# KrArunT/whisper-rust-ort

Measured on AMD Instinct MI355X. Metric: rtfx: audio seconds transcribed per wall second (whisper-base, 30 s clips, greedy 128 new tokens), higher is better.
Workload: dtype bf16

## Files before the change

### whisper-rust-ort_amd/build.py

```python
from __future__ import annotations

import os
import subprocess
import sys
from concurrent.futures import ThreadPoolExecutor

HERE = os.path.dirname(os.path.abspath(__file__))
CSRC = os.path.join(HERE, "csrc")
OUT = os.path.join(HERE, "libwhisper_hip.so")
SOURCES = ["wh_mel.hip", "wh_gemm.hip", "wh_gemm8.hip", "wh_gemm8x.hip", "wh_gemm8_mx.hip", "wh_mlp.hip", "wh_attn.hip", "wh_decode.hip", "wh_dec_tile.hip", "wh_cross_es.hip", "wh_cross_es8.hip", "wh_cross_es3.hip", "wh_fp8.hip", "wh_align.hip", "wh_model.cpp", "wh_api.cpp"]
HEADERS = ["wh_common.h", "wh_es_common.h", "wh_kernels.h", "wh_lm_tile.h", "wh_internal.h", "wh_json.h", "../../include/whisper_hip.h"]
FLAGS = ["--offload-arch=gfx950", "-O3", "-fPIC", "-std=c++17", "-pthread", "-Wall", "-Wno-unused-function", "-Wno-unused-value", "-Wno-unused-result",
         "-mllvm", "-amdgpu-mfma-vgpr-form=1", "-x", "hip"]


EXTRA_FLAGS = {"wh_attn.hip": ["-fno-honor-nans"], "wh_cross_es.hip": ["-fno-honor-nans"], "wh_cross_es8.hip": ["-fno-honor-nans"], "wh_cross_es3.hip": ["-fno-honor-nans"]}


def _stale(target: str, deps) -> bool:
    if not os.path.exists(target):
        return True
    t = os.path.getmtime(target)
    return any(os.path.getmtime(d) > t for d in deps)


def build(verbose: bool = False, force: bool = False) -> str:
    hipcc = os.environ.get("HIPCC", "/opt/rocm/bin/hipcc")
    objdir = os.path.join(HERE, "build")
    os.makedirs(objdir, exist_ok=True)
    hdrs = [os.path.join(CSRC, h) for h in HEADERS]

    def compile_one(src: str) -> str:
        s = os.path.join(CSRC, src)
        o = os.path.join(objdir, src + ".o")
        if force or _stale(o, [s] + hdrs):
            cmd = [hipcc] + FLAGS + EXTRA_FLAGS.get(src, []) + ["-c", s, "-o", o]
            if verbose:
                print(" ".join(cmd), flush=True)
            subprocess.check_call(cmd)
        return o

    with ThreadPoolExecutor(max_workers=min(6, os.cpu_count() or 1)) as ex:
        objs = list(ex.map(compile_one, SOURCES))
    if force or _stale(OUT, objs):
        cmd = [hipcc, "--offload-arch=gfx950", "-shared", "-fPIC", "-pthread", "-o", OUT] + objs
        if verbose:
            print(" ".join(cmd), flush=True)
        subprocess.check_call(cmd)
    build_host(verbose, force)
    build_tools(verbose, force)
    return OUT


TOOLS = os.path.join(HERE, "..", "tools")


def build_tools(verbose: bool = False, force: bool = False) -> None:
    hipcc = os.environ.get("HIPCC", "/opt/rocm/bin/hipcc")
    for name, kernel_src in (("mx_mfma_check", "wh_gemm8_mx.hip"), ("mx_gemm_check", "wh_gemm8_mx.hip"), ("mlp_check", "wh_mlp.hip"), ("es16_check", "wh_cross_es.hip"), ("es8_check", "wh_cross_es8.hip"), ("es3_check", "wh_cross_es3.hip"), ("align_check", "wh_align.hip")):
        src, exe = os.path.join(TOOLS, name + ".hip"), os.path.join(TOOLS, name)
        deps = [src, os.path.join(CSRC, kernel_src), os.path.join(CSRC, "wh_common.h"), os.path.join(CSRC, "wh_es_common.h"), os.path.join(CSRC, "wh_kernels.h")]
        if force or _stale(exe, deps):
            cmd = [hipcc, "--offload-arch=gfx950", "-O3", "-std=c++17", "-mllvm", "-amdgpu-mfma-vgpr-form=1"] + EXTRA_FLAGS.get(kernel_src, []) + ["-w", "-I", CSRC, src, "-o", exe]
            if verbose:
                print(" ".join(cmd), flush=True)
            subprocess.check_call(cmd)


HOST = os.path.join(HERE, "host")
HOST_SO = os.path.join(HERE, "libwh_host.so")
CLI = os.path.join(HERE, "whisper_bench")


def build_host(verbose: bool = False, force: bool = False) -> None:
    gxx = os.environ.get("CXX", "g++")
    hdr = [os.path.join(HOST, "wh_host.h"), os.path.join(HOST, "wh_unicode_lower.h"), os.path.join(CSRC, "wh_json.h"), os.path.join(HERE, "..", "include", "whisper_hip.h")]
    src = os.path.join(HOST, "wh_host_capi.cpp")
    if force or _stale(HOST_SO, [src] + hdr):
        cmd = [gxx, "-O2", "-std=c++17", "-fPIC", "-shared", "-Wall", "-o", HOST_SO, src]
        if verbose:
            print(" ".join(cmd), flush=True)
        subprocess.check_call(cmd)
    src = os.path.join(HOST, "whisper_bench.cpp")
    if force or _stale(CLI, [src, OUT] + hdr):
        cmd = [gxx, "-O2", "-std=c++17", "-Wall", "-pthread", "-D__HIP_PLATFORM_AMD__", "-I/opt/rocm/include", "-o", CLI, src, "-L" + HERE, "-lwhisper_hip",
               "-Wl,-rpath,$ORIGIN", "-Wl,-rpath,/opt/rocm/lib", "-L/opt/rocm/lib", "-lamdhip64"]
        if verbose:
            print(" ".join(cmd), flush=True)
        subprocess.check_call(cmd)


if __name__ == "__main__":
    print(build(verbose=True, force="--force" in sys.argv))
```

### whisper-rust-ort_amd/csrc/wh_decode.hip

```cpp
#include <stdlib.h>

#include "wh_common.h"
#include "wh_kernels.h"

#include <algorithm>
#include <mutex>
#include <unordered_map>

int wh_dbg_cross_unroll = 4;
int wh_dbg_lm_blocks_per_cu = 2;
int wh_dbg_lm_mt = 4;
int wh_dbg_mt = 0;
int wh_dbg_nw = 0;
int wh_dbg_wide = -1;

namespace {

__device__ __forceinline__ void advance_if_last(int* ticket, int* pos_p, int n_blocks) {
    if (!ticket) return;
    __syncthreads();
    if (threadIdx.x == 0) {
        const int t = atomicAdd(ticket, 1);
        if (t == n_blocks - 1) {
            *ticket = 0;
// ... 895 lines not shown
    const int fl = lane & 15, fg = lane >> 4;
    const int n_tiles = (a.n_lang + 15) >> 4;
    const int m0 = blockIdx.y * MT * 16;
    T* Xs = reinterpret_cast<T*>(smem_raw);
    constexpr int ROWS = MT * 16;
    const int nslab = a.K >> 5, cps = ROWS * 32 / EPC;
    u32x4 xr[16];
    int xo[16];
    auto stage_load = [&](int c0) {
#pragma unroll
        for (int i = 0; i < 16; i++) {
            const int c = min(c0 + i * 256, nslab * cps - 1), sl = c / cps, o = (c - sl * cps) * EPC;
            xo[i] = sl * ROWS * 32 + o;
            xr[i] = *reinterpret_cast<const u32x4*>((const T*)a.X + ((long)sl * a.x_mpad + m0) * 32 + o);
        }
    };
    auto stage_store = [&](int c0) {
#pragma unroll
        for (int i = 0; i < 16; i++)
            if (c0 + i * 256 < nslab * cps) *reinterpret_cast<u32x4*>(Xs + xo[i]) = xr[i];
    };
    stage_load(tid);
    float* lnstat = reinterpret_cast<float*>(smem_raw + (size_t)nslab * ROWS * 32 * sizeof(T));
    {
        float* lnq = lnstat + 2 * ROWS;
        if (tid < 4 * ROWS) {
            const int r = tid % ROWS, q = tid / ROWS;
            float s1, s2;
            ln_partial_sum(a.ln_part, a.ln_tiles, a.x_mpad, m0 + r, q, 4, s1, s2);
            lnq[(q * ROWS + r) * 2] = s1;
            lnq[(q * ROWS + r) * 2 + 1] = s2;
        }
        __syncthreads();
        if (tid < ROWS) {
            const float s1 = (lnq[tid * 2] + lnq[(ROWS + tid) * 2]) + (lnq[(2 * ROWS + tid) * 2] + lnq[(3 * ROWS + tid) * 2]);
            const float s2 = (lnq[tid * 2 + 1] + lnq[(ROWS + tid) * 2 + 1]) + (lnq[(2 * ROWS + tid) * 2 + 1] + lnq[(3 * ROWS + tid) * 2 + 1]);
            float mean, rstd;
            wh_ln_mean_rstd(s1, s2, (float)a.K, false, mean, rstd);
            lnstat[2 * tid] = mean;
            lnstat[2 * tid + 1] = rstd;
        }
    }
    const int iters = a.K >> 5;
    constexpr int DEPTH = sizeof(typename FragT<T>::type) <= 16 ? 16 : 8;
    const int nchunk = (iters + DEPTH - 1) / DEPTH;
    const int tile = blockIdx.x * 4 + wave;
    const int units = tile < n_tiles ? nchunk : 0;
    typedef typename FragT<T>::type frag_t;
    frag_t wA[DEPTH], wB[DEPTH];
    f32x4 acc[MT];
#pragma unroll
    for (int t = 0; t < MT; t++) acc[t] = f32x4{0, 0, 0, 0};
    const T* wp = (const T*)a.W + (long)a.ids[min(tile, WH_LANG_LD / 16 - 1) * 16 + fl] * a.K + fg * 8;
    auto load_unit = [&](frag_t (&wq)[DEPTH], int u) {
#pragma unroll
        for (int i = 0; i < DEPTH; i++)
            if (u * DEPTH + i < iters) wq[i] = load_frag<T>(wp + (u * DEPTH + i) * 32);
    };
    auto compute_unit = [&](const frag_t (&wq)[DEPTH], int u) {
#pragma unroll
        for (int i = 0; i < DEPTH; i++) {
            if (u * DEPTH + i < iters) {
#pragma unroll
                for (int t = 0; t < MT; t++) {
                    frag_t xf = load_frag<T>(Xs + ((long)(u * DEPTH + i) * ROWS + t * 16 + fl) * 32 + fg * 8);
                    mma16(acc[t], wq[i], xf);
                }
            }
        }
    };
    if (units > 0) load_unit(wA, 0);
    stage_store(tid);
    for (int c0 = tid + 256 * 16; c0 < nslab * cps; c0 += 256 * 16) {
        stage_load(c0);
        stage_store(c0);
    }
    __syncthreads();
    for (int u = 0; u < units; u += 2) {
        const bool hasB = u + 1 < units;
        if (hasB) load_unit(wB, u + 1);
        compute_unit(wA, u);
        if (hasB) {
            if (u + 2 < units) load_unit(wA, u + 2);
            compute_unit(wB, u + 1);
        }
    }
    if (units == 0) return;
    const int j0 = tile * 16 + 4 * fg;
    float sv[4] = {0, 0, 0, 0}, cv[4] = {0, 0, 0, 0};
#pragma unroll
    for (int e = 0; e < 4; e++) {
        const int id = a.ids[j0 + e];
        sv[e] = a.ln_s[id];
        cv[e] = a.bias[id];
    }
#pragma unroll
    for (int t = 0; t < MT; t++) {
        const int m = m0 + t * 16 + fl;
        const float mean = lnstat[2 * (t * 16 + fl)], rstd = lnstat[2 * (t * 16 + fl) + 1];
        f32x4 v;
#pragma unroll
        for (int e = 0; e < 4; e++) v[e] = wh_ln_fold(acc[t][e], mean, rstd, sv[e], cv[e]);
        if (m < a.M) *reinterpret_cast<f32x4*>(a.out + (long)m * WH_LANG_LD + j0) = v;
    }
}

__global__ __launch_bounds__(64) void k_lang_finish(const float* __restrict__ logits, const int* __restrict__ ids, int n_lang, int src_row,
                                                    float* __restrict__ probs, int* __restrict__ chosen, int* __restrict__ feed,
                                                    int* __restrict__ out_tokens, int tok_ld, int tok_pos, int* pos_p) {
    const int b = blockIdx.x, lane = threadIdx.x;
    const float* row = logits + (long)(src_row >= 0 ? src_row : b) * WH_LANG_LD;
    float v[2];
    int id[2];
    float bv = -INFINITY;
    int bi = 0x7fffffff, lo = 0x7fffffff;
#pragma unroll
    for (int k = 0; k < 2; k++) {
        const int j = lane + 64 * k;
        const bool in = j < n_lang;
        v[k] = in ? row[j] : NAN;
        id[k] = in ? ids[j] : 0x7fffffff;
        lo = min(lo, id[k]);
        if (v[k] > bv || (v[k] == bv && id[k] < bi)) { bv = v[k]; bi = id[k]; }
    }
#pragma unroll
    for (int off = 32; off > 0; off >>= 1) {
        const float ov = __shfl_xor(bv, off);
        const int oi = __shfl_xor(bi, off), ol = __shfl_xor(lo, off);
        if (ov > bv || (ov == bv && oi < bi)) { bv = ov; bi = oi; }
        lo = min(lo, ol);
    }
    const bool none = bv == -INFINITY;
    float e[2], s = 0.0f;
#pragma unroll
    for (int k = 0; k < 2; k++) {
        e[k] = (none || !(v[k] == v[k])) ? 0.0f : (bv == INFINITY ? (v[k] == INFINITY ? 1.0f : 0.0f) : ts_exp(v[k] - bv));
        s += e[k];
    }
    s = wave_sum(s);
#pragma unroll
    for (int k = 0; k < 2; k++) {
        const int j = lane + 64 * k;
        if (j < n_lang) probs[(long)b * n_lang + j] = none ? 0.0f : e[k] / s;
    }
    if (lane == 0) {
        const int tok = none ? lo : bi;
        chosen[b] = tok;
        feed[(long)b * tok_ld + tok_pos] = tok;
        out_tokens[(long)b * tok_ld + tok_pos] = tok;
        if (pos_p && b == 0) *pos_p += 1;
    }
}

template <typename T, typename TO = T, bool PFX = false>
__global__ __launch_bounds__(64) void k_dec_self_attn(const T* __restrict__ qkv, T* __restrict__ kc,
                                                      T* __restrict__ vc, TO* __restrict__ out,
                                                      const int* __restrict__ pos_p, int d, int n_heads, int tc_plane,
                                                      int mpad, const int* __restrict__ off) {
    constexpr int HD = WH_HEAD_DIM;
    typedef typename FragT<T>::type frag_t;
    __shared__ __attribute__((aligned(16))) float qs[HD];
    __shared__ __attribute__((aligned(16))) float sc[512];
    const int h = blockIdx.x, b = blockIdx.y, lane = threadIdx.x, gpos = *pos_p;
    int adv = 0;
    if constexpr (PFX) adv = min(max(off[b], 0), gpos);
    const int pos = gpos - adv, tc = tc_plane - adv;
    const T* row = qkv + (long)b * 3 * d;
    T* kcb = kc + (((long)b * n_heads + h) * tc_plane + adv) * HD;
    T* vcb = vc + (((long)b * n_heads + h) * tc_plane + adv) * HD;
    frag_t kr[2][HD / 8];
#pragma unroll
    for (int i = 0; i < 2; i++) {
        const int j = lane + 64 * i;
        if (j < pos) {
#pragma unroll
            for (int e = 0; e < HD / 8; e++) kr[i][e] = load_frag<T>(kcb + (long)j * HD + e * 8);
        }
    }
    constexpr int EPC = 16 / (int)sizeof(T), CPR = HD / EPC, RPI = 64 / CPR, NPRE = 8;
    typedef __attribute__((ext_vector_type(EPC))) T vrow_t;
    const int rslot = lane / CPR, chunk = lane % CPR;
    vrow_t vpre[NPRE];
#pragma unroll
    for (int u = 0; u < NPRE; u++)
        vpre[u] = *reinterpret_cast<const vrow_t*>(vcb + (long)min(u * RPI + rslot, tc - 1) * HD + chunk * EPC);
    const vrow_t vcur_v = *reinterpret_cast<const vrow_t*>(row + 2 * d + h * HD + chunk * EPC);
    const T kcur = row[d + h * HD + lane], vcur = row[2 * d + h * HD + lane];
    qs[lane] = cvt_in<T>(row[h * HD + lane]);
    kcb[(long)pos * HD + lane] = kcur;
    vcb[(long)pos * HD + lane] = vcur;
    __syncthreads();
    float mx = -INFINITY;
#pragma unroll
    for (int i = 0; i < 2; i++) {
        const int j = lane + 64 * i;
        if (j < pos) {
            float s = 0.0f;
#pragma unroll
            for (int e = 0; e < HD / 8; e++)
#pragma unroll
                for (int u = 0; u < 8; u++) s += qs[e * 8 + u] * (float)kr[i][e][u];
            sc[j] = s;
            mx = fmaxf(mx, s);
        }
    }
    for (int j = lane + 128; j < pos; j += 64) {
        float s = 0.0f;
#pragma unroll
        for (int e = 0; e < HD / 8; e++) {
            const frag_t kk = load_frag<T>(kcb + (long)j * HD + e * 8);
#pragma unroll
            for (int u = 0; u < 8; u++) s += qs[e * 8 + u] * (float)kk[u];
        }
        sc[j] = s;
        mx = fmaxf(mx, s);
    }
    const float scur = dpp_wave_sum(qs[lane] * cvt_in<T>(kcur));
    mx = fmaxf(dpp_wave_max(mx), scur);
    float sum = 0.0f;
    for (int j = lane; j < pos; j += 64) {
        const float p = __expf(sc[j] - mx);
        sc[j] = p;
        sum += p;
    }
    const float pcur = __expf(scur - mx);
    sum = dpp_wave_sum(sum) + pcur;
    __syncthreads();
    float o[EPC];
#pragma unroll
    for (int e = 0; e < EPC; e++) o[e] = (rslot == 0) ? pcur * cvt_in<T>(vcur_v[e]) : 0.0f;
#pragma unroll
    for (int u = 0; u < NPRE; u++) {
        const int r = u * RPI + rslot;
        const float pr = (r < pos) ? sc[min(r, 511)] : 0.0f;
#pragma unroll
        for (int e = 0; e < EPC; e++) o[e] += (r < pos) ? pr * cvt_in<T>(vpre[u][e]) : 0.0f;
    }
    for (int j = NPRE * RPI; j < pos; j += NPRE * RPI) {
        vrow_t v[NPRE];
#pragma unroll
        for (int u = 0; u < NPRE; u++)
            v[u] = *reinterpret_cast<const vrow_t*>(vcb + (long)min(j + u * RPI + rslot, tc - 1) * HD + chunk * EPC);
#pragma unroll
        for (int u = 0; u < NPRE; u++) {
            const int r = j + u * RPI + rslot;
            const float pr = (r < pos) ? sc[min(r, 511)] : 0.0f;
#pragma unroll
            for (int e = 0; e < EPC; e++) o[e] += (r < pos) ? pr * cvt_in<T>(v[u][e]) : 0.0f;
        }
    }
#pragma unroll
    for (int e = 0; e < EPC; e++) {
        float t = o[e];
        if (CPR == 8) t += __builtin_bit_cast(float, __builtin_amdgcn_update_dpp(0, __builtin_bit_cast(int, t), 0x128, 0xF, 0xF, true));
        o[e] = xrow_sum(t);
    }
    if (rslot == 0) {
        const float inv = 1.0f / sum;
        if constexpr (EPC == 4) {
            store4(out + slab_idx(b, h * HD + chunk * EPC, mpad), o[0] * inv, o[1] * inv, o[2] * inv, o[3] * inv);
        } else {
            vrow_t ov;
#pragma unroll
            for (int e = 0; e < EPC; e++) ov[e] = cvt_out<T>(o[e] * inv);
            *reinterpret_cast<vrow_t*>(out + slab_idx(b, h * HD + chunk * EPC, mpad)) = ov;
        }
    }
}

template <typename T, int NCH, int UNROLL, bool NT, typename TO = T>
__global__ __launch_bounds__(256) void k_dec_cross_attn(const T* __restrict__ q, const T* __restrict__ ck,
                                                        const T* __restrict__ cv, float* __restrict__ part,
                                                        float* __restrict__ ml, int S, int d, int n_heads,
                                                        int splits, TO* __restrict__ out, int mpad) {
    constexpr int EPC = 16 / (int)sizeof(T);
    constexpr int LPH = WH_HEAD_DIM / EPC;
    extern __shared__ __attribute__((aligned(16))) float smem[];
    typedef __attribute__((ext_vector_type(EPC))) T vec_t;
    const int tid = threadIdx.x, lane = tid & 63, wave = tid >> 6;
    const int sp = blockIdx.x, b = blockIdx.y;
    const int per = (S + splits - 1) / splits;
    const int ks = sp * per, ke = min(S, ks + per);
    const int j1 = ke;
    const int chunks = d / EPC;

    constexpr bool PACKED = sizeof(T) == 2;
    float qv[NCH][EPC], o[NCH][EPC], mrun[NCH], lrun[NCH];
    wh_u32x4 qd[NCH];
#pragma unroll
    for (int c = 0; c < NCH; c++) {
        const int ch = lane + 64 * c;
        mrun[c] = -INFINITY;
        lrun[c] = 0.0f;
        qd[c] = wh_u32x4{0, 0, 0, 0};
        if (PACKED && ch < chunks) qd[c] = *reinterpret_cast<const wh_u32x4*>(q + (long)b * d + ch * EPC);
#pragma unroll
        for (int u = 0; u < EPC; u++) {
            qv[c][u] = (!PACKED && ch < chunks) ? cvt_in<T>(q[(long)b * d + ch * EPC + u]) : 0.0f;
            o[c][u] = 0.0f;
        }
    }
    const T* kb = ck + (long)b * S * d;
    const T* vb = cv + (long)b * S * d;
    vec_t kA[UNROLL][NCH], vA[UNROLL][NCH], kB[UNROLL][NCH], vB[UNROLL][NCH];
    auto load_set = [&](vec_t (&kk)[UNROLL][NCH], vec_t (&vv)[UNROLL][NCH], int j) {
#pragma unroll
        for (int u = 0; u < UNROLL; u++) {
            const int jj = min(j + u, j1 - 1);
#pragma unroll
            for (int c = 0; c < NCH; c++) {
                const int ch = lane + 64 * c;
                if (ch < chunks) {
                    if constexpr (NT) {
                        kk[u][c] = __builtin_nontemporal_load(reinterpret_cast<const vec_t*>(kb + (long)jj * d + ch * EPC));
                        vv[u][c] = __builtin_nontemporal_load(reinterpret_cast<const vec_t*>(vb + (long)jj * d + ch * EPC));
                    } else {
                        kk[u][c] = *reinterpret_cast<const vec_t*>(kb + (long)jj * d + ch * EPC);
                        vv[u][c] = *reinterpret_cast<const vec_t*>(vb + (long)jj * d + ch * EPC);
                    }
                }
            }
        }
    };
    auto compute_set = [&](const vec_t (&kk)[UNROLL][NCH], const vec_t (&vv)[UNROLL][NCH], int j) {
#pragma unroll
        for (int c = 0; c < NCH; c++) {
            const int ch = lane + 64 * c;
            float s[UNROLL];
            float mx = mrun[c];
#pragma unroll
            for (int u = 0; u < UNROLL; u++) {
                float t = 0.0f;
                if (ch < chunks) {
                    if constexpr (PACKED) {
                        t = dot8_bf16(as_u32x4(kk[u][c]), qd[c], t);
                    } else {
#pragma unroll
                        for (int e = 0; e < EPC; e++) t += qv[c][e] * (float)kk[u][c][e];
                    }
                }
                t = dpp_group_sum<LPH>(t);
                s[u] = (j + u < j1) ? t : -INFINITY;
                mx = fmaxf(mx, s[u]);
            }
            const float scale = __expf(mrun[c] - mx);
            float ls = lrun[c] * scale;
#pragma unroll
            for (int e = 0; e < EPC; e++) o[c][e] *= scale;
            if constexpr (PACKED && (UNROLL % 2 == 0)) {
#pragma unroll
                for (int u = 0; u < UNROLL; u += 2) {
                    const float p0 = __expf(s[u] - mx), p1 = __expf(s[u + 1] - mx);
                    ls += p0 + p1;
                    const bf16x2 pp = bf16x2{(bf16)p0, (bf16)p1};
                    if (ch < chunks) {
                        const wh_u32x4 va = as_u32x4(vv[u][c]), vb = as_u32x4(vv[u + 1][c]);
                        pv2_bf16(va.x, vb.x, pp, o[c][0], o[c][1]);
                        pv2_bf16(va.y, vb.y, pp, o[c][2], o[c][3]);
                        pv2_bf16(va.z, vb.z, pp, o[c][4], o[c][5]);
                        pv2_bf16(va.w, vb.w, pp, o[c][6], o[c][7]);
                    }
                }
            } else {
#pragma unroll
                for (int u = 0; u < UNROLL; u++) {
                    const float p = __expf(s[u] - mx);
                    ls += p;
                    if (ch < chunks) {
#pragma unroll
                        for (int e = 0; e < EPC; e++) o[c][e] += p * (float)vv[u][c][e];
                    }
                }
            }
            mrun[c] = mx;
            lrun[c] = ls;
        }
    };
    constexpr int GS = 4 * UNROLL;
    const int j0 = ks + wave * UNROLL;
    if (j0 < j1) load_set(kA, vA, j0);
    for (int j = j0; j < j1; j += 2 * GS) {
        const bool hasB = j + GS < j1;
        if (hasB) load_set(kB, vB, j + GS);
        compute_set(kA, vA, j);
        if (hasB) {
            if (j + 2 * GS < j1) load_set(kA, vA, j + 2 * GS);
            compute_set(kB, vB, j + GS);
        }
    }
    float* wm = smem;
    float* wl = wm + 4 * n_heads;
    float* wo = wl + 4 * n_heads;
#pragma unroll
    for (int c = 0; c < NCH; c++) {
        const int ch = lane + 64 * c;
        if (ch < chunks) {
            if ((lane % LPH) == 0) {
                wm[wave * n_heads + ch / LPH] = mrun[c];
                wl[wave * n_heads + ch / LPH] = lrun[c];
            }
#pragma unroll
            for (int e = 0; e < EPC; e++) wo[wave * d + ch * EPC + e] = o[c][e];
        }
    }
    __syncthreads();
    float* pp = part + ((long)b * splits + sp) * d;
    float* mp = ml + ((long)b * splits + sp) * n_heads * 2;
    for (int n = tid; n < d; n += 256) {
        const int h = n / WH_HEAD_DIM;
        const float M = fmaxf(fmaxf(wm[h], wm[n_heads + h]), fmaxf(wm[2 * n_heads + h], wm[3 * n_heads + h]));
        float num = 0.0f, den = 0.0f;
#pragma unroll
        for (int w = 0; w < 4; w++) {
            const float mw = wm[w * n_heads + h];
            const float sc = (mw == -INFINITY) ? 0.0f : __expf(mw - M);
            num += sc * wo[w * d + n];
            den += sc * wl[w * n_heads + h];
        }
        if (out) {
            store1(out + slab_idx(b, n, mpad), num / den);
            continue;
        }
// ... 130 lines not shown
        const int rg = (a.M + 16 * WMT - 1) / (16 * WMT);
        int nt = 1;
        if (NW == 4 && n_tiles % 4 == 0 && (n_tiles / 4) * rg * a.zn >= 512) nt = 4;
        else if (n_tiles % 2 == 0 && (n_tiles / 2) * rg * a.zn >= 128) nt = 2;
        if (wide == 2 || (wide == 4 && NW == 4)) nt = wide;
        if (wide != 0 && nt > 1 && n_tiles % nt == 0) {
            const size_t smw = (size_t)NW * WMT * nt * 64 * 16 + (size_t)4 * WMT * 16 * 2 * 4;
            dim3 gw(n_tiles / nt, rg, a.zn);
            if (nt == 4) { set_max_smem(k_dec_gemm_wide<T, TO, WMT, 4, NW, TW>, smw); hipLaunchKernelGGL((k_dec_gemm_wide<T, TO, WMT, 4, NW, TW>), gw, dim3(NW * 64), smw, s, a); }
            else { set_max_smem(k_dec_gemm_wide<T, TO, WMT, 2, NW, TW>, smw); hipLaunchKernelGGL((k_dec_gemm_wide<T, TO, WMT, 2, NW, TW>), gw, dim3(NW * 64), smw, s, a); }
            return;
        }
    }
    const int mt = std::min(mt_cap, (a.M + 15) / 16);
    const size_t sm = (size_t)NW * mt * 64 * 16 + (size_t)4 * mt * 16 * 2 * 4;
    dim3 grid(n_tiles, (a.M + 16 * mt - 1) / (16 * mt), a.zn);
    if (a.xpart) {
        dim3 g1(n_tiles, (a.M + 15) / 16);
        const size_t sm1 = (size_t)NW * 64 * 16 + 4 * 16 * 2 * 4 + (size_t)16 * a.K * sizeof(T);
        if (a.x_splits <= 4) { set_max_smem(k_dec_gemm<T, TO, 1, NW, 4, TW>, sm1); hipLaunchKernelGGL((k_dec_gemm<T, TO, 1, NW, 4, TW>), g1, dim3(NW * 64), sm1, s, a); }
        else if (a.x_splits <= 8) { set_max_smem(k_dec_gemm<T, TO, 1, NW, 8, TW>, sm1); hipLaunchKernelGGL((k_dec_gemm<T, TO, 1, NW, 8, TW>), g1, dim3(NW * 64), sm1, s, a); }
        else if (a.x_splits <= 16) { set_max_smem(k_dec_gemm<T, TO, 1, NW, 16, TW>, sm1); hipLaunchKernelGGL((k_dec_gemm<T, TO, 1, NW, 16, TW>), g1, dim3(NW * 64), sm1, s, a); }
        else { set_max_smem(k_dec_gemm<T, TO, 1, NW, 32, TW>, sm1); hipLaunchKernelGGL((k_dec_gemm<T, TO, 1, NW, 32, TW>), g1, dim3(NW * 64), sm1, s, a); }
        return;
    }
    switch (mt) {
        case 1: hipLaunchKernelGGL((k_dec_gemm<T, TO, 1, NW, 0, TW>), grid, dim3(NW * 64), sm, s, a); break;
        case 2: hipLaunchKernelGGL((k_dec_gemm<T, TO, 2, NW, 0, TW>), grid, dim3(NW * 64), sm, s, a); break;
        case 3: hipLaunchKernelGGL((k_dec_gemm<T, TO, 3, NW, 0, TW>), grid, dim3(NW * 64), sm, s, a); break;
        default: hipLaunchKernelGGL((k_dec_gemm<T, TO, 4, NW, 0, TW>), grid, dim3(NW * 64), sm, s, a); break;
    }
}

static inline bool dec_gemm_8way(const SkinnyArgs& a) {
    return (a.K >= 2048 || a.xpart || (a.K >= 1024 && a.N <= 4096)) && a.K % 256 == 0;
}

template <typename T, typename TO, typename TW>
void launch_dec_gemm_split(hipStream_t s, const SkinnyArgs& a) {
    const bool eight = wh_dbg_nw ? (wh_dbg_nw == 8 && a.K % 256 == 0) : dec_gemm_8way(a);
    if (eight) launch_dec_gemm_mt<T, TO, 8, TW>(s, a);
    else launch_dec_gemm_mt<T, TO, 4, TW>(s, a);
}

}

void wh_launch_dec_gemm(hipStream_t s, int prec, bool out_f32, const SkinnyArgs& a) {
    if (prec == WH_PREC_F32) launch_dec_gemm_split<float, float, float>(s, a);
    else if (prec == WH_PREC_F16X3) launch_dec_gemm_split<h2, float, h2>(s, a);
    else if (prec == WH_PREC_FP8 && a.wscale) {
        const int nw = dec_gemm_8way(a) ? 8 : 4;
        const bool wide = (a.K / nw) % 64 == 0;
        if (wide) { if (out_f32) launch_dec_gemm_split<bf16, float, fp8x16_t>(s, a); else launch_dec_gemm_split<bf16, bf16, fp8x16_t>(s, a); }
        else { if (out_f32) launch_dec_gemm_split<bf16, float, fp8x8_t>(s, a); else launch_dec_gemm_split<bf16, bf16, fp8x8_t>(s, a); }
    } else if (out_f32) launch_dec_gemm_split<bf16, float, bf16>(s, a);
    else launch_dec_gemm_split<bf16, bf16, bf16>(s, a);
}

void wh_launch_dec_embed(hipStream_t s, int prec, const void* tok_emb, const float* pos_emb, const int* feed, int feed_ld,
                         const int* pos_p, float* x, void* xslab, float* stats, int rows, int d, int mpad, const float* xgamma, float* shift, const int* off) {
    dim3 grid((rows + 3) / 4);
    wh_with_dtype(prec, [&](auto tag) {
        typedef typename decltype(tag)::type T;
        wh_with_flags([&](auto PFX) {
            hipLaunchKernelGGL((k_dec_embed<T, decltype(PFX)::value>), grid, dim3(256), 0, s, (const T*)tok_emb, pos_emb, feed, feed_ld, pos_p, x, (T*)xslab, stats, rows, d, mpad, xgamma, shift, off);
        }, off != nullptr);
    });
}

template <typename T>
static dim3 lm_head_geometry(const SkinnyArgs& a, int* mt_out, size_t* sm_out) {
    const int n_tiles = (a.N + 15) / 16;
    int mt = std::min(wh_dbg_lm_mt, (a.M + 15) / 16);
    auto lds = [&](int t) { return (size_t)t * 16 * a.K * sizeof(T) + (size_t)t * 16 * 2 * 4 * 5; };
    while (mt > 1 && lds(mt) > 150 * 1024) mt--;
    if (mt > 4) mt = 4;
    const size_t sm = lds(mt);
    const int per_cu = std::max<int>(1, (int)(150 * 1024 / sm));
    *mt_out = mt;
    *sm_out = sm;
    return dim3(std::min((n_tiles + 3) / 4, 256 * std::min(per_cu, wh_dbg_lm_blocks_per_cu) / ((a.M + 16 * mt - 1) / (16 * mt))), (a.M + 16 * mt - 1) / (16 * mt));
}

template <typename T>
static void launch_lm_head_v(hipStream_t s, const SkinnyArgs& a) {
    int mt;
    size_t sm;
    const dim3 grid = lm_head_geometry<T>(a, &mt, &sm);
    wh_with_flags([&](auto RULES, auto LP, auto REP) {
        wh_with_1to4(mt, [&](auto MT) {
            auto kfn = k_lm_head<T, decltype(MT)::value, decltype(RULES)::value, decltype(LP)::value, decltype(REP)::value>;
            set_max_smem(kfn, sm);
            hipLaunchKernelGGL(kfn, grid, dim3(256), sm, s, a);
        });
    }, a.ts_logits != nullptr, a.part_sum != nullptr, a.rep_bits != nullptr);
}
void wh_launch_lm_head(hipStream_t s, int prec, const SkinnyArgs& a) {
    if (prec == WH_PREC_F32) launch_lm_head_v<float>(s, a);
    else if (prec == WH_PREC_F16X3) {
        if (wh_lm_head_tile_x3_applicable(a)) wh_launch_lm_head_tile_x3(s, a);
        else launch_lm_head_v<h2>(s, a);
    }
    else if (wh_lm_head_tile_applicable(a)) wh_launch_lm_head_tile(s, a);
    else launch_lm_head_v<bf16>(s, a);
}

int wh_lm_head_parts(int prec, const SkinnyArgs& a) {
    int mt;
    size_t sm;
    if (prec == WH_PREC_F16X3 && wh_lm_head_tile_x3_applicable(a)) return wh_lm_head_tile_x3_parts(a);
    if (prec == WH_PREC_F32 || prec == WH_PREC_F16X3) return (int)lm_head_geometry<float>(a, &mt, &sm).x * 4;
    if (wh_lm_head_tile_applicable(a)) return wh_lm_head_tile_parts(a);
    return (int)lm_head_geometry<bf16>(a, &mt, &sm).x * 4;
}

void wh_launch_argmax_finish(hipStream_t s, int prec, const float* part_val, const int* part_idx, int n_parts, int mpad, int* pos_p,
                             int* ticket, const DecodeState& st, int B, const NextEmbed& ne, const TsFinish& ts, const float* part_sum, const RepFinish& rp) {
    wh_with_dtype(prec, [&](auto tag) {
        typedef typename decltype(tag)::type T;
        wh_with_flags([&](auto RULES, auto LP, auto PFX, auto REP) {
            hipLaunchKernelGGL((k_argmax_finish<T, decltype(RULES)::value, decltype(LP)::value, decltype(PFX)::value, decltype(REP)::value>), dim3(B), dim3(256), 0, s,
                               part_val, part_idx, n_parts, mpad, pos_p, ticket, st, ne, ts, part_sum, rp);
        }, ts.rules, part_sum != nullptr, ne.tok_emb && ne.off, rp.on);
    });
}

void wh_launch_nospeech_finish(hipStream_t s, const float* part_val, const float* part_sum, int n_parts, int mpad, const float* probe_v,
                               float* prob, int B, int* pos_p) {
    hipLaunchKernelGGL(k_nospeech_finish, dim3(B), dim3(64), 0, s, part_val, part_sum, n_parts, mpad, probe_v, prob, pos_p);
}

template <typename T>
static void launch_lang_head_t(hipStream_t s, const LangHeadArgs& a) {
    int mt = std::min(wh_dbg_lm_mt, (a.M + 15) / 16);
    auto lds = [&](int t) { return (size_t)t * 16 * a.K * sizeof(T) + (size_t)t * 16 * 2 * 4 * 5; };
    while (mt > 1 && lds(mt) > 150 * 1024) mt--;
    if (mt > 4) mt = 4;
    const size_t sm = lds(mt);
    dim3 grid(((a.n_lang + 15) / 16 + 3) / 4, (a.M + 16 * mt - 1) / (16 * mt));
    wh_with_1to4(mt, [&](auto MT) {
        auto kfn = k_lang_head<T, decltype(MT)::value>;
        set_max_smem(kfn, sm);
        hipLaunchKernelGGL(kfn, grid, dim3(256), sm, s, a);
    });
}

void wh_launch_lang_head(hipStream_t s, int prec, const LangHeadArgs& a) {
    wh_with_dtype(prec, [&](auto tag) { launch_lang_head_t<typename decltype(tag)::type>(s, a); });
}

void wh_launch_lang_finish(hipStream_t s, const float* logits, const int* ids, int n_lang, int src_row, float* probs, int* chosen, int* feed,
                           int* out_tokens, int tok_ld, int tok_pos, int B, int* pos_p) {
    hipLaunchKernelGGL(k_lang_finish, dim3(B), dim3(64), 0, s, logits, ids, n_lang, src_row, probs, chosen, feed, out_tokens, tok_ld, tok_pos, pos_p);
}

void wh_launch_dec_self_attn(hipStream_t s, int prec, const void* qkv, void* kc, void* vc, void* out, const int* pos_p,
                             int d, int n_heads, int tc, int B, int mpad, const int* off) {
    dim3 grid(n_heads, B);
    wh_with_flags([&](auto pfx) {
        constexpr bool PFX = decltype(pfx)::value;
        if (prec == WH_PREC_F16X3)
            hipLaunchKernelGGL((k_dec_self_attn<float, h2, PFX>), grid, dim3(64), 0, s, (const float*)qkv, (float*)kc, (float*)vc, (h2*)out, pos_p, d, n_heads, tc, mpad, off);
        else if (prec == WH_PREC_F32)
            hipLaunchKernelGGL((k_dec_self_attn<float, float, PFX>), grid, dim3(64), 0, s, (const float*)qkv, (float*)kc, (float*)vc, (float*)out, pos_p, d, n_heads, tc, mpad, off);
        else
            hipLaunchKernelGGL((k_dec_self_attn<bf16, bf16, PFX>), grid, dim3(64), 0, s, (const bf16*)qkv, (bf16*)kc, (bf16*)vc, (bf16*)out, pos_p, d, n_heads, tc, mpad, off);
    }, off != nullptr);
}

size_t wh_cross_lds_reserve(long total_wgs, size_t own_bytes) {
    static const int cap = [] { const char* e = getenv("WH_CROSS_WGS_PER_CU"); return e ? atoi(e) : 2; }();
    if (cap <= 0 || cap > 2 || total_wgs <= (long)cap * 256) return own_bytes;
    const size_t target = cap == 1 ? (size_t)150 * 1024 : (size_t)72 * 1024;
    return own_bytes > target ? own_bytes : target;
}

void wh_launch_dec_cross_attn(hipStream_t s, int prec, const void* q, const void* ck, const void* cv, float* part,
                              float* ml, int S, int d, int n_heads, int splits, int B, void* out, int mpad, bool stream_nt) {
    dim3 grid(splits, B);
    const bool f32_layout = prec == WH_PREC_F32 || prec == WH_PREC_F16X3;
    const long wgs = (long)splits * B * ((!f32_layout && d > 512 && d % 256 == 0) ? d / 256 : 1);
    const size_t sm = wh_cross_lds_reserve(wgs, sizeof(float) * ((size_t)8 * n_heads + 4 * (size_t)d));
#define WH_CA2(T_, N_, U_, NT_, TO_) do { set_max_smem(k_dec_cross_attn<T_, N_, U_, NT_, TO_>, sm);                                                 \
                                     hipLaunchKernelGGL((k_dec_cross_attn<T_, N_, U_, NT_, TO_>), grid, dim3(256), sm, s, (const T_*)q, (const T_*)ck, \
                                             (const T_*)cv, part, ml, S, d, n_heads, splits, (TO_*)(splits == 1 ? out : nullptr), mpad); } while (0)
#define WH_CA1(T_, N_, U_, NT_) WH_CA2(T_, N_, U_, NT_, T_)
    static const int nt_env = [] { const char* e = getenv("WH_CROSS_NT"); return e ? atoi(e) : -1; }();
    if (nt_env >= 0) stream_nt = nt_env != 0;
#define WH_CA(T_, N_, U_) do { if (stream_nt) WH_CA1(T_, N_, U_, true); else WH_CA1(T_, N_, U_, false); } while (0)
    if (prec == WH_PREC_F16X3) {
#define WH_CAX(N_, U_) do { if (stream_nt) WH_CA2(float, N_, U_, true, h2); else WH_CA2(float, N_, U_, false, h2); } while (0)
        const int nch = (d / 4 + 63) / 64;
        if (nch == 1) WH_CAX(1, 4);
        else if (nch == 2) WH_CAX(2, 2);
        else WH_CAX(5, 1);
#undef WH_CAX
    } else if (f32_layout) {
        const int nch = (d / 4 + 63) / 64;
        if (nch == 1) WH_CA(float, 1, 4);
        else if (nch == 2) WH_CA(float, 2, 2);
        else WH_CA(float, 5, 1);
    } else {
        const int nch = (d / 8 + 63) / 64;
        static const int unroll_env = [] { const char* e = getenv("WH_CROSS_UNROLL"); return e ? atoi(e) : 0; }();
        if (nch == 1) {
            const int un = unroll_env ? unroll_env : wh_dbg_cross_unroll;
            if (un == 8) WH_CA(bf16, 1, 8);
            else if (un == 2) WH_CA(bf16, 1, 2);
            else WH_CA(bf16, 1, 4);
        }
        else if (d % 256 == 0 && getenv("WH_CROSS_ALLHEADS") == nullptr) {
            dim3 g3(splits, B, d / 256);
            bf16* o = (bf16*)(splits == 1 ? out : nullptr);
            const size_t smcg = wh_cross_lds_reserve(wgs, 12 * 1024) - 12 * 1024;
            if (stream_nt) { set_max_smem(k_dec_cross_attn_cg<4, true>, smcg); hipLaunchKernelGGL((k_dec_cross_attn_cg<4, true>), g3, dim3(256), smcg, s, (const bf16*)q, (const bf16*)ck, (const bf16*)cv, part, ml, S, d, n_heads, splits, o, mpad); }
            else { set_max_smem(k_dec_cross_attn_cg<4, false>, smcg); hipLaunchKernelGGL((k_dec_cross_attn_cg<4, false>), g3, dim3(256), smcg, s, (const bf16*)q, (const bf16*)ck, (const bf16*)cv, part, ml, S, d, n_heads, splits, o, mpad); }
        } else WH_CA(bf16, 3, 2);
    }
#undef WH_CA
#undef WH_CA1
#undef WH_CA2
}
```

Before: 73170.

## Add LDS-ring pipelined decoder self-attention kernel and make it default for bf16

Moves decoder self-attention into its own file and adds a variant that streams K rows into a swizzled LDS ring buffer via global_load_lds, with vmcnt-based waits so loads overlap the QK dot products. V rows are double-buffered in registers. This variant is now the default for bf16, while the original kernel stays as a fallback with an optional LIVE mode that skips loads past pos. The goal is to hide K/V cache load latency during per-token decode, at the cost of more LDS use and hand-written asm waits that could be fragile.

```diff
diff --git a/whisper-rust-ort_amd/build.py b/whisper-rust-ort_amd/build.py
--- a/whisper-rust-ort_amd/build.py
+++ b/whisper-rust-ort_amd/build.py
@@ -8,7 +8,7 @@
 HERE = os.path.dirname(os.path.abspath(__file__))
 CSRC = os.path.join(HERE, "csrc")
 OUT = os.path.join(HERE, "libwhisper_hip.so")
-SOURCES = ["wh_mel.hip", "wh_gemm.hip", "wh_gemm8.hip", "wh_gemm8x.hip", "wh_gemm8_mx.hip", "wh_mlp.hip", "wh_attn.hip", "wh_decode.hip", "wh_dec_tile.hip", "wh_cross_es.hip", "wh_cross_es8.hip", "wh_cross_es3.hip", "wh_fp8.hip", "wh_align.hip", "wh_model.cpp", "wh_api.cpp"]
+SOURCES = ["wh_mel.hip", "wh_gemm.hip", "wh_gemm8.hip", "wh_gemm8x.hip", "wh_gemm8_mx.hip", "wh_mlp.hip", "wh_attn.hip", "wh_decode.hip", "wh_self_attn.hip", "wh_dec_tile.hip", "wh_cross_es.hip", "wh_cross_es8.hip", "wh_cross_es3.hip", "wh_fp8.hip", "wh_align.hip", "wh_model.cpp", "wh_api.cpp"]
 HEADERS = ["wh_common.h", "wh_es_common.h", "wh_kernels.h", "wh_lm_tile.h", "wh_internal.h", "wh_json.h", "../../include/whisper_hip.h"]
 FLAGS = ["--offload-arch=gfx950", "-O3", "-fPIC", "-std=c++17", "-pthread", "-Wall", "-Wno-unused-function", "-Wno-unused-value", "-Wno-unused-result",
          "-mllvm", "-amdgpu-mfma-vgpr-form=1", "-x", "hip"]
@@ -57,7 +57,7 @@
 
 def build_tools(verbose: bool = False, force: bool = False) -> None:
     hipcc = os.environ.get("HIPCC", "/opt/rocm/bin/hipcc")
-    for name, kernel_src in (("mx_mfma_check", "wh_gemm8_mx.hip"), ("mx_gemm_check", "wh_gemm8_mx.hip"), ("mlp_check", "wh_mlp.hip"), ("es16_check", "wh_cross_es.hip"), ("es8_check", "wh_cross_es8.hip"), ("es3_check", "wh_cross_es3.hip"), ("align_check", "wh_align.hip")):
+    for name, kernel_src in (("mx_mfma_check", "wh_gemm8_mx.hip"), ("mx_gemm_check", "wh_gemm8_mx.hip"), ("mlp_check", "wh_mlp.hip"), ("es16_check", "wh_cross_es.hip"), ("es8_check", "wh_cross_es8.hip"), ("es3_check", "wh_cross_es3.hip"), ("align_check", "wh_align.hip"), ("self_attn_check", "wh_self_attn.hip")):
         src, exe = os.path.join(TOOLS, name + ".hip"), os.path.join(TOOLS, name)
         deps = [src, os.path.join(CSRC, kernel_src), os.path.join(CSRC, "wh_common.h"), os.path.join(CSRC, "wh_es_common.h"), os.path.join(CSRC, "wh_kernels.h")]
         if force or _stale(exe, deps):
diff --git a/whisper-rust-ort_amd/csrc/wh_decode.hip b/whisper-rust-ort_amd/csrc/wh_decode.hip
--- a/whisper-rust-ort_amd/csrc/wh_decode.hip
+++ b/whisper-rust-ort_amd/csrc/wh_decode.hip
@@ -1071,122 +1071,6 @@
     }
 }
 
-template <typename T, typename TO = T, bool PFX = false>
-__global__ __launch_bounds__(64) void k_dec_self_attn(const T* __restrict__ qkv, T* __restrict__ kc,
-                                                      T* __restrict__ vc, TO* __restrict__ out,
-                                                      const int* __restrict__ pos_p, int d, int n_heads, int tc_plane,
-                                                      int mpad, const int* __restrict__ off) {
-    constexpr int HD = WH_HEAD_DIM;
-    typedef typename FragT<T>::type frag_t;
-    __shared__ __attribute__((aligned(16))) float qs[HD];
-    __shared__ __attribute__((aligned(16))) float sc[512];
-    const int h = blockIdx.x, b = blockIdx.y, lane = threadIdx.x, gpos = *pos_p;
-    int adv = 0;
-    if constexpr (PFX) adv = min(max(off[b], 0), gpos);
-    const int pos = gpos - adv, tc = tc_plane - adv;
-    const T* row = qkv + (long)b * 3 * d;
-    T* kcb = kc + (((long)b * n_heads + h) * tc_plane + adv) * HD;
-    T* vcb = vc + (((long)b * n_heads + h) * tc_plane + adv) * HD;
-    frag_t kr[2][HD / 8];
-#pragma unroll
-    for (int i = 0; i < 2; i++) {
-        const int j = lane + 64 * i;
-        if (j < pos) {
-#pragma unroll
-            for (int e = 0; e < HD / 8; e++) kr[i][e] = load_frag<T>(kcb + (long)j * HD + e * 8);
-        }
-    }
-    constexpr int EPC = 16 / (int)sizeof(T), CPR = HD / EPC, RPI = 64 / CPR, NPRE = 8;
-    typedef __attribute__((ext_vector_type(EPC))) T vrow_t;
-    const int rslot = lane / CPR, chunk = lane % CPR;
-    vrow_t vpre[NPRE];
-#pragma unroll
-    for (int u = 0; u < NPRE; u++)
-        vpre[u] = *reinterpret_cast<const vrow_t*>(vcb + (long)min(u * RPI + rslot, tc - 1) * HD + chunk * EPC);
-    const vrow_t vcur_v = *reinterpret_cast<const vrow_t*>(row + 2 * d + h * HD + chunk * EPC);
-    const T kcur = row[d + h * HD + lane], vcur = row[2 * d + h * HD + lane];
-    qs[lane] = cvt_in<T>(row[h * HD + lane]);
-    kcb[(long)pos * HD + lane] = kcur;
-    vcb[(long)pos * HD + lane] = vcur;
-    __syncthreads();
-    float mx = -INFINITY;
-#pragma unroll
-    for (int i = 0; i < 2; i++) {
-        const int j = lane + 64 * i;
-        if (j < pos) {
-            float s = 0.0f;
-#pragma unroll
-            for (int e = 0; e < HD / 8; e++)
-#pragma unroll
-                for (int u = 0; u < 8; u++) s += qs[e * 8 + u] * (float)kr[i][e][u];
-            sc[j] = s;
-            mx = fmaxf(mx, s);
-        }
-    }
-    for (int j = lane + 128; j < pos; j += 64) {
-        float s = 0.0f;
-#pragma unroll
-        for (int e = 0; e < HD / 8; e++) {
-            const frag_t kk = load_frag<T>(kcb + (long)j * HD + e * 8);
-#pragma unroll
-            for (int u = 0; u < 8; u++) s += qs[e * 8 + u] * (float)kk[u];
-        }
-        sc[j] = s;
-        mx = fmaxf(mx, s);
-    }
-    const float scur = dpp_wave_sum(qs[lane] * cvt_in<T>(kcur));
-    mx = fmaxf(dpp_wave_max(mx), scur);
-    float sum = 0.0f;
-    for (int j = lane; j < pos; j += 64) {
-        const float p = __expf(sc[j] - mx);
-        sc[j] = p;
-        sum += p;
-    }
-    const float pcur = __expf(scur - mx);
-    sum = dpp_wave_sum(sum) + pcur;
-    __syncthreads();
-    float o[EPC];
-#pragma unroll
-    for (int e = 0; e < EPC; e++) o[e] = (rslot == 0) ? pcur * cvt_in<T>(vcur_v[e]) : 0.0f;
-#pragma unroll
-    for (int u = 0; u < NPRE; u++) {
-        const int r = u * RPI + rslot;
-        const float pr = (r < pos) ? sc[min(r, 511)] : 0.0f;
-#pragma unroll
-        for (int e = 0; e < EPC; e++) o[e] += (r < pos) ? pr * cvt_in<T>(vpre[u][e]) : 0.0f;
-    }
-    for (int j = NPRE * RPI; j < pos; j += NPRE * RPI) {
-        vrow_t v[NPRE];
-#pragma unroll
-        for (int u = 0; u < NPRE; u++)
-            v[u] = *reinterpret_cast<const vrow_t*>(vcb + (long)min(j + u * RPI + rslot, tc - 1) * HD + chunk * EPC);
-#pragma unroll
-        for (int u = 0; u < NPRE; u++) {
-            const int r = j + u * RPI + rslot;
-            const float pr = (r < pos) ? sc[min(r, 511)] : 0.0f;
-#pragma unroll
-            for (int e = 0; e < EPC; e++) o[e] += (r < pos) ? pr * cvt_in<T>(v[u][e]) : 0.0f;
-        }
-    }
-#pragma unroll
-    for (int e = 0; e < EPC; e++) {
-        float t = o[e];
-        if (CPR == 8) t += __builtin_bit_cast(float, __builtin_amdgcn_update_dpp(0, __builtin_bit_cast(int, t), 0x128, 0xF, 0xF, true));
-        o[e] = xrow_sum(t);
-    }
-    if (rslot == 0) {
-        const float inv = 1.0f / sum;
-        if constexpr (EPC == 4) {
-            store4(out + slab_idx(b, h * HD + chunk * EPC, mpad), o[0] * inv, o[1] * inv, o[2] * inv, o[3] * inv);
-        } else {
-            vrow_t ov;
-#pragma unroll
-            for (int e = 0; e < EPC; e++) ov[e] = cvt_out<T>(o[e] * inv);
-            *reinterpret_cast<vrow_t*>(out + slab_idx(b, h * HD + chunk * EPC, mpad)) = ov;
-        }
-    }
-}
-
 template <typename T, int NCH, int UNROLL, bool NT, typename TO = T>
 __global__ __launch_bounds__(256) void k_dec_cross_attn(const T* __restrict__ q, const T* __restrict__ ck,
                                                         const T* __restrict__ cv, float* __restrict__ part,
@@ -1623,20 +1507,6 @@
 void wh_launch_lang_finish(hipStream_t s, const float* logits, const int* ids, int n_lang, int src_row, float* probs, int* chosen, int* feed,
                            int* out_tokens, int tok_ld, int tok_pos, int B, int* pos_p) {
     hipLaunchKernelGGL(k_lang_finish, dim3(B), dim3(64), 0, s, logits, ids, n_lang, src_row, probs, chosen, feed, out_tokens, tok_ld, tok_pos, pos_p);
-}
-
-void wh_launch_dec_self_attn(hipStream_t s, int prec, const void* qkv, void* kc, void* vc, void* out, const int* pos_p,
-                             int d, int n_heads, int tc, int B, int mpad, const int* off) {
-    dim3 grid(n_heads, B);
-    wh_with_flags([&](auto pfx) {
-        constexpr bool PFX = decltype(pfx)::value;
-        if (prec == WH_PREC_F16X3)
-            hipLaunchKernelGGL((k_dec_self_attn<float, h2, PFX>), grid, dim3(64), 0, s, (const float*)qkv, (float*)kc, (float*)vc, (h2*)out, pos_p, d, n_heads, tc, mpad, off);
-        else if (prec == WH_PREC_F32)
-            hipLaunchKernelGGL((k_dec_self_attn<float, float, PFX>), grid, dim3(64), 0, s, (const float*)qkv, (float*)kc, (float*)vc, (float*)out, pos_p, d, n_heads, tc, mpad, off);
-        else
-            hipLaunchKernelGGL((k_dec_self_attn<bf16, bf16, PFX>), grid, dim3(64), 0, s, (const bf16*)qkv, (bf16*)kc, (bf16*)vc, (bf16*)out, pos_p, d, n_heads, tc, mpad, off);
-    }, off != nullptr);
 }
 
 size_t wh_cross_lds_reserve(long total_wgs, size_t own_bytes) {
diff --git a/whisper-rust-ort_amd/csrc/wh_self_attn.hip b/whisper-rust-ort_amd/csrc/wh_self_attn.hip
--- /dev/null
+++ b/whisper-rust-ort_amd/csrc/wh_self_attn.hip
@@ -0,0 +1,308 @@
+#include <stdlib.h>
+
+#include "wh_common.h"
+#include "wh_kernels.h"
+
+int wh_dbg_self_attn_form = -1;
+
+namespace {
+
+typedef const __attribute__((address_space(1))) void* gptr_t;
+typedef __attribute__((address_space(3))) void* lptr_t;
+
+__device__ __forceinline__ long slab_idx(int m, int k, int mpad) { return ((long)(k >> 5) * mpad + m) * 32 + (k & 31); }
+
+template <int N> __device__ __forceinline__ void wait_vm() { asm volatile("s_waitcnt vmcnt(%0)" ::"n"(N) : "memory"); }
+__device__ __forceinline__ void glds16(const void* src, char* lds_wave_base) {
+    __builtin_amdgcn_global_load_lds((gptr_t)src, (lptr_t)lds_wave_base, 16, 0, 0);
+}
+
+template <int CPR> __device__ __forceinline__ int kswz(int r) { return CPR == 8 ? (r >> 1) & 7 : r & 15; }
+__device__ __forceinline__ bf16x8 ring_frag(const bf16* rowp, int e, int key) {
+    return *reinterpret_cast<const bf16x8*>(reinterpret_cast<const char*>(rowp) + ((e ^ key) << 4));
+}
+__device__ __forceinline__ f32x8 ring_frag(const float* rowp, int e, int key) {
+    const f32x4 a = *reinterpret_cast<const f32x4*>(reinterpret_cast<const char*>(rowp) + (((2 * e) ^ key) << 4));
+    const f32x4 b = *reinterpret_cast<const f32x4*>(reinterpret_cast<const char*>(rowp) + (((2 * e + 1) ^ key) << 4));
+    return f32x8{a[0], a[1], a[2], a[3], b[0], b[1], b[2], b[3]};
+}
+
+template <typename T, typename TO = T, bool PFX = false>
+__global__ __launch_bounds__(64) void k_dec_self_attn_lds(const T* __restrict__ qkv, T* __restrict__ kc,
+                                                      T* __restrict__ vc, TO* __restrict__ out,
+                                                      const int* __restrict__ pos_p, int d, int n_heads, int tc_plane,
+                                                      int mpad, const int* __restrict__ off) {
+    constexpr int HD = WH_HEAD_DIM;
+    typedef typename FragT<T>::type frag_t;
+    constexpr int EPC = 16 / (int)sizeof(T), CPR = HD / EPC, RPI = 64 / CPR;
+    constexpr int PPR = 64 / RPI;
+    constexpr int NP = 2 * PPR + 1;
+    constexpr int NT = 8;
+    typedef __attribute__((ext_vector_type(EPC))) T vrow_t;
+    __shared__ __attribute__((aligned(16))) float qs[HD];
+    __shared__ __attribute__((aligned(16))) float sc[512];
+    __shared__ __attribute__((aligned(256))) char kring[NP * 1024];
+    const int h = blockIdx.x, b = blockIdx.y, lane = threadIdx.x, gpos = *pos_p;
+    int adv = 0;
+    if constexpr (PFX) adv = min(max(off[b], 0), gpos);
+    const int pos = gpos - adv;
+    const T* row = qkv + (long)b * 3 * d;
+    T* kcb = kc + (((long)b * n_heads + h) * tc_plane + adv) * HD;
+    T* vcb = vc + (((long)b * n_heads + h) * tc_plane + adv) * HD;
+    const int rslot = lane / CPR, chunk = lane % CPR;
+    auto k_piece = [&](int q) {
+        const int r = q * RPI + rslot;
+        glds16(kcb + (long)min(r, pos - 1) * HD + (chunk ^ kswz<CPR>(r)) * EPC, kring + (q % NP) * 1024);
+    };
+    auto v_group = [&](int g) {
+        return *reinterpret_cast<const vrow_t*>(vcb + (long)min(g * RPI + rslot, pos - 1) * HD + chunk * EPC);
+    };
+#pragma unroll
+    for (int q = 0; q < NP; q++)
+        if (q * RPI < pos) k_piece(q);
+    vrow_t vpre[NP];
+#pragma unroll
+    for (int u = 0; u < NP; u++)
+        if (u * RPI < pos) vpre[u] = v_group(u);
+    const vrow_t vcur_v = *reinterpret_cast<const vrow_t*>(row + 2 * d + h * HD + chunk * EPC);
+    const T kcur = row[d + h * HD + lane], vcur = row[2 * d + h * HD + lane];
+    qs[lane] = cvt_in<T>(row[h * HD + lane]);
+    wait_vm<0>();
+    __syncthreads();
+    float mx = -INFINITY;
+    for (int i = 0; i * 64 < pos; i++) {
+        if (i > 0) {
+            if ((NP + PPR * i - 1) * RPI < pos) wait_vm<PPR>();
+            else wait_vm<0>();
+        }
+        const int j = lane + 64 * i;
+        if (j < pos) {
+            const T* kr = reinterpret_cast<const T*>(kring + ((j / RPI) % NP) * 1024) + (j % RPI) * HD;
+            const int key = kswz<CPR>(j);
+            float s = 0.0f;
+#pragma unroll
+            for (int e = 0; e < HD / 8; e++) {
+                const frag_t kk = ring_frag(kr, e, key);
+#pragma unroll
+                for (int u = 0; u < 8; u++) s += qs[e * 8 + u] * (float)kk[u];
+            }
+            sc[j] = s;
+            mx = fmaxf(mx, s);
+        }
+        if ((NP + PPR * i) * RPI < pos) {
+            asm volatile("s_waitcnt lgkmcnt(0)" ::: "memory");
+#pragma unroll
+            for (int t = 0; t < PPR; t++) {
+                const int q = NP + PPR * i + t;
+                if (q * RPI < pos) k_piece(q);
+            }
+        }
+    }
+    kcb[(long)pos * HD + lane] = kcur;
+    vcb[(long)pos * HD + lane] = vcur;
+    const int ngrp = (pos + RPI - 1) / RPI;
+    vrow_t vA[NT], vB[NT];
+    auto v_set = [&](vrow_t (&v)[NT], int g0) {
+#pragma unroll
+        for (int u = 0; u < NT; u++)
+            if (g0 + u < ngrp) v[u] = v_group(g0 + u);
+    };
+    if (NP < ngrp) v_set(vA, NP);
+    const float scur = dpp_wave_sum(qs[lane] * cvt_in<T>(kcur));
+    mx = fmaxf(dpp_wave_max(mx), scur);
+    float sum = 0.0f;
+    for (int j = lane; j < pos; j += 64) {
+        const float p = __expf(sc[j] - mx);
+        sc[j] = p;
+        sum += p;
+    }
+    const float pcur = __expf(scur - mx);
+    sum = dpp_wave_sum(sum) + pcur;
+    __syncthreads();
+    float o[EPC];
+#pragma unroll
+    for (int e = 0; e < EPC; e++) o[e] = (rslot == 0) ? pcur * cvt_in<T>(vcur_v[e]) : 0.0f;
+    auto pv = [&](const vrow_t& v, int g) {
+        const int r = g * RPI + rslot;
+        const float pr = (r < pos) ? sc[min(r, 511)] : 0.0f;
+#pragma unroll
+        for (int e = 0; e < EPC; e++) o[e] += (r < pos) ? pr * cvt_in<T>(v[e]) : 0.0f;
+    };
+    auto pv_set = [&](const vrow_t (&v)[NT], int g0) {
+#pragma unroll
+        for (int u = 0; u < NT; u++)
+            if (g0 + u < ngrp) pv(v[u], g0 + u);
+    };
+#pragma unroll
+    for (int u = 0; u < NP; u++)
+        if (u * RPI < pos) pv(vpre[u], u);
+    for (int g0 = NP; g0 < ngrp; g0 += 2 * NT) {
+        const bool hasB = g0 + NT < ngrp;
+        if (hasB) v_set(vB, g0 + NT);
+        pv_set(vA, g0);
+        if (hasB) {
+            if (g0 + 2 * NT < ngrp) v_set(vA, g0 + 2 * NT);
+            pv_set(vB, g0 + NT);
+        }
+    }
+#pragma unroll
+    for (int e = 0; e < EPC; e++) {
+        float t = o[e];
+        if (CPR == 8) t += __builtin_bit_cast(float, __builtin_amdgcn_update_dpp(0, __builtin_bit_cast(int, t), 0x128, 0xF, 0xF, true));
+        o[e] = xrow_sum(t);
+    }
+    if (rslot == 0) {
+        const float inv = 1.0f / sum;
+        if constexpr (EPC == 4) {
+            store4(out + slab_idx(b, h * HD + chunk * EPC, mpad), o[0] * inv, o[1] * inv, o[2] * inv, o[3] * inv);
+        } else {
+            vrow_t ov;
+#pragma unroll
+            for (int e = 0; e < EPC; e++) ov[e] = cvt_out<T>(o[e] * inv);
+            *reinterpret_cast<vrow_t*>(out + slab_idx(b, h * HD + chunk * EPC, mpad)) = ov;
+        }
+    }
+}
+
+template <typename T, typename TO = T, bool PFX = false, bool LIVE = false>
+__global__ __launch_bounds__(64) void k_dec_self_attn(const T* __restrict__ qkv, T* __restrict__ kc,
+                                                         T* __restrict__ vc, TO* __restrict__ out,
+                                                         const int* __restrict__ pos_p, int d, int n_heads, int tc_plane,
+                                                         int mpad, const int* __restrict__ off) {
+    constexpr int HD = WH_HEAD_DIM;
+    typedef typename FragT<T>::type frag_t;
+    __shared__ __attribute__((aligned(16))) float qs[HD];
+    __shared__ __attribute__((aligned(16))) float sc[512];
+    const int h = blockIdx.x, b = blockIdx.y, lane = threadIdx.x, gpos = *pos_p;
+    int adv = 0;
+    if constexpr (PFX) adv = min(max(off[b], 0), gpos);
+    const int pos = gpos - adv, tc = tc_plane - adv;
+    const T* row = qkv + (long)b * 3 * d;
+    T* kcb = kc + (((long)b * n_heads + h) * tc_plane + adv) * HD;
+    T* vcb = vc + (((long)b * n_heads + h) * tc_plane + adv) * HD;
+    frag_t kr[2][HD / 8];
+#pragma unroll
+    for (int i = 0; i < 2; i++) {
+        const int j = lane + 64 * i;
+        if (j < pos) {
+#pragma unroll
+            for (int e = 0; e < HD / 8; e++) kr[i][e] = load_frag<T>(kcb + (long)j * HD + e * 8);
+        }
+    }
+    constexpr int EPC = 16 / (int)sizeof(T), CPR = HD / EPC, RPI = 64 / CPR, NPRE = 8;
+    typedef __attribute__((ext_vector_type(EPC))) T vrow_t;
+    const int rslot = lane / CPR, chunk = lane % CPR;
+    vrow_t vpre[NPRE];
+#pragma unroll
+    for (int u = 0; u < NPRE; u++)
+        if (!LIVE || u * RPI < pos) vpre[u] = *reinterpret_cast<const vrow_t*>(vcb + (long)min(u * RPI + rslot, LIVE ? pos - 1 : tc - 1) * HD + chunk * EPC);
+    const vrow_t vcur_v = *reinterpret_cast<const vrow_t*>(row + 2 * d + h * HD + chunk * EPC);
+    const T kcur = row[d + h * HD + lane], vcur = row[2 * d + h * HD + lane];
+    qs[lane] = cvt_in<T>(row[h * HD + lane]);
+    kcb[(long)pos * HD + lane] = kcur;
+    vcb[(long)pos * HD + lane] = vcur;
+    __syncthreads();
+    float mx = -INFINITY;
+#pragma unroll
+    for (int i = 0; i < 2; i++) {
+        const int j = lane + 64 * i;
+        if (j < pos) {
+            float s = 0.0f;
+#pragma unroll
+            for (int e = 0; e < HD / 8; e++)
+#pragma unroll
+                for (int u = 0; u < 8; u++) s += qs[e * 8 + u] * (float)kr[i][e][u];
+            sc[j] = s;
+            mx = fmaxf(mx, s);
+        }
+    }
+    for (int j = lane + 128; j < pos; j += 64) {
+        float s = 0.0f;
+#pragma unroll
+        for (int e = 0; e < HD / 8; e++) {
+            const frag_t kk = load_frag<T>(kcb + (long)j * HD + e * 8);
+#pragma unroll
+            for (int u = 0; u < 8; u++) s += qs[e * 8 + u] * (float)kk[u];
+        }
+        sc[j] = s;
+        mx = fmaxf(mx, s);
+    }
+    const float scur = dpp_wave_sum(qs[lane] * cvt_in<T>(kcur));
+    mx = fmaxf(dpp_wave_max(mx), scur);
+    float sum = 0.0f;
+    for (int j = lane; j < pos; j += 64) {
+        const float p = __expf(sc[j] - mx);
+        sc[j] = p;
+        sum += p;
+    }
+    const float pcur = __expf(scur - mx);
+    sum = dpp_wave_sum(sum) + pcur;
+    __syncthreads();
+    float o[EPC];
+#pragma unroll
+    for (int e = 0; e < EPC; e++) o[e] = (rslot == 0) ? pcur * cvt_in<T>(vcur_v[e]) : 0.0f;
+#pragma unroll
+    for (int u = 0; u < NPRE; u++) {
+        if (LIVE && u * RPI >= pos) continue;
+        const int r = u * RPI + rslot;
+        const float pr = (r < pos) ? sc[min(r, 511)] : 0.0f;
+#pragma unroll
+        for (int e = 0; e < EPC; e++) o[e] += (r < pos) ? pr * cvt_in<T>(vpre[u][e]) : 0.0f;
+    }
+    for (int j = NPRE * RPI; j < pos; j += NPRE * RPI) {
+        vrow_t v[NPRE];
+#pragma unroll
+        for (int u = 0; u < NPRE; u++)
+            if (!LIVE || j + u * RPI < pos) v[u] = *reinterpret_cast<const vrow_t*>(vcb + (long)min(j + u * RPI + rslot, LIVE ? pos - 1 : tc - 1) * HD + chunk * EPC);
+#pragma unroll
+        for (int u = 0; u < NPRE; u++) {
+            if (LIVE && j + u * RPI >= pos) continue;
+            const int r = j + u * RPI + rslot;
+            const float pr = (r < pos) ? sc[min(r, 511)] : 0.0f;
+#pragma unroll
+            for (int e = 0; e < EPC; e++) o[e] += (r < pos) ? pr * cvt_in<T>(v[u][e]) : 0.0f;
+        }
+    }
+#pragma unroll
+    for (int e = 0; e < EPC; e++) {
+        float t = o[e];
+        if (CPR == 8) t += __builtin_bit_cast(float, __builtin_amdgcn_update_dpp(0, __builtin_bit_cast(int, t), 0x128, 0xF, 0xF, true));
+        o[e] = xrow_sum(t);
+    }
+    if (rslot == 0) {
+        const float inv = 1.0f / sum;
+        if constexpr (EPC == 4) {
+            store4(out + slab_idx(b, h * HD + chunk * EPC, mpad), o[0] * inv, o[1] * inv, o[2] * inv, o[3] * inv);
+        } else {
+            vrow_t ov;
+#pragma unroll
+            for (int e = 0; e < EPC; e++) ov[e] = cvt_out<T>(o[e] * inv);
+            *reinterpret_cast<vrow_t*>(out + slab_idx(b, h * HD + chunk * EPC, mpad)) = ov;
+        }
+    }
+}
+
+}
+
+void wh_launch_dec_self_attn(hipStream_t s, int prec, const void* qkv, void* kc, void* vc, void* out, const int* pos_p,
+                             int d, int n_heads, int tc, int B, int mpad, const int* off) {
+    static const int env_form = [] {
+        const char* v1 = getenv("WH_SELF_ATTN_V1");
+        const char* lds = getenv("WH_SELF_ATTN_LDS");
+        const char* live = getenv("WH_SELF_ATTN_LIVE");
+        return (v1 && atoi(v1) != 0) ? 1 : (lds && atoi(lds) != 0) ? 0 : (live && atoi(live) != 0) ? 2 : -1;
+    }();
+    int form = wh_dbg_self_attn_form >= 0 ? wh_dbg_self_attn_form : env_form;
+    if (form < 0) form = (prec == WH_PREC_F32 || prec == WH_PREC_F16X3) ? 1 : 0;
+    dim3 grid(n_heads, B);
+    wh_with_flags([&](auto pfx, auto live, auto lds) {
+        constexpr bool PFX = decltype(pfx)::value, LIVE = decltype(live)::value, LDS = decltype(lds)::value;
+        auto launch = [&](auto kfn, auto* q, auto* k, auto* v, auto* o) { hipLaunchKernelGGL(kfn, grid, dim3(64), 0, s, q, k, v, o, pos_p, d, n_heads, tc, mpad, off); };
+        if (prec == WH_PREC_F16X3)
+            launch(LDS ? k_dec_self_attn_lds<float, h2, PFX> : k_dec_self_attn<float, h2, PFX, LIVE>, (const float*)qkv, (float*)kc, (float*)vc, (h2*)out);
+        else if (prec == WH_PREC_F32)
+            launch(LDS ? k_dec_self_attn_lds<float, float, PFX> : k_dec_self_attn<float, float, PFX, LIVE>, (const float*)qkv, (float*)kc, (float*)vc, (float*)out);
+        else
+            launch(LDS ? k_dec_self_attn_lds<bf16, bf16, PFX> : k_dec_self_attn<bf16, bf16, PFX, LIVE>, (const bf16*)qkv, (bf16*)kc, (bf16*)vc, (bf16*)out);
+    }, off != nullptr, form == 2, form == 0);
+}
```

Result: no change. 73710, median of 6 (+0.7%).
